# AmandineBtto/NeRAF

Measured on AMD Instinct MI355X. Metric: field-samples/sec (rays + RIR STFT bins), higher is better.
Workload: dtype f16; 1 GPU; RAF FurnishedRoom joint training step (BASELINE configs[2]): 4096 rays + 2048 RIR slices x 513 bins per GPU; radiance + grid refresh + ResNet3D + NAcF + STFT loss, backward, GradScaler + fused Adam...; rays_per_gpu=4096, slices_per_gpu=2048, global_rays=4096, global_slices=2048, parallelism=dp1, distinct_resident_batches=16, deterministic=True

## Files before the change

include/neraf_hip.h:

```cpp
#ifndef NERAF_HIP_H
#define NERAF_HIP_H

#include <stddef.h>
#include <stdint.h>

#ifdef __cplusplus
extern "C" {
#endif

typedef struct neraf_ctx neraf_ctx;
typedef void* neraf_stream_t;

enum {
  NERAF_OK = 0,
  NERAF_EINVAL = -1,
  NERAF_EHIP = -2,
  NERAF_ENOGPU = -3,
  NERAF_ESTATE = -4
};

#define NERAF_ABI_VERSION 1

int neraf_abi_version(void);
int neraf_ctx_create(neraf_ctx** out, int device);
// ... 238 lines not shown
                           const float* g_reg, float* d_pose, neraf_stream_t stream);

int neraf_loss_sum_scale(neraf_ctx* ctx, const float* const* terms, int n, const float* scale, float* out2, neraf_stream_t stream);
int neraf_vision_loss_finalize(neraf_ctx* ctx, const float* sums, const float* k3, float* out4, neraf_stream_t stream);
int neraf_vision_bwd_prologue(neraf_ctx* ctx, const float* u_rgb, const float* u_dens, const float* u_dist, const float* g_rgb,
                              const float* g_inter, const float* g_dist, size_t n_samples, float* d_rgb, float* d_dens, float* up3,
                              float* d_rays, size_t n_ray_floats, float* sums4, neraf_stream_t stream);

int neraf_cvt_f16_segments(neraf_ctx* ctx, const float* const* src, void* const* dst, const long long* len, int n,
                           neraf_stream_t stream);
int neraf_gather_f16(neraf_ctx* ctx, const float* const* src, const long long* src_len, int nsrc, const long long* index, void* dst,
                     long long n, neraf_stream_t stream);

int neraf_resnet3d_debug_locate(const neraf_resnet3d_desc* d, int kind, int index, size_t* offset, int* rows, int* cols);

uint32_t neraf_debug_fastdiv(uint32_t n, uint32_t d);

int neraf_fused_adam_chunk(void);
int neraf_grads_nonfinite(neraf_ctx* ctx, const void* table, const void* g_ptrs, const int* blk_tensor, const int* blk_chunk,
                          int n_blocks, float* found_inf, const void* const* g_ptrs_host, int n_ptrs, int found_is_zero,
                          neraf_stream_t stream);
int neraf_amp_update_scale(neraf_ctx* ctx, float* scale, int32_t* growth_tracker, const float* const* found_infs, int n,
                           double growth_factor, double backoff_factor, int growth_interval, int clear_flags, neraf_stream_t stream);
int neraf_fused_adam(neraf_ctx* ctx, const void* table, const void* g_ptrs, const int* blk_tensor, const int* blk_chunk,
                     int n_blocks, const float* group_lr, int n_groups, int n_tensors, double beta1, double beta2, double eps,
                     float* step, const float* grad_scale, const float* found_inf, neraf_stream_t stream);

int neraf_fused_adam_dual(neraf_ctx* ctx, const void* table, const void* g_ptrs, const int* blk_tensor, const int* blk_chunk,
                          int n_blocks, const float* group_lr, int n_groups, int n_tensors, double beta1, double beta2, double eps,
                          float* step, const float* grad_scale, const float* found_inf, const void* dual, const float* step0,
// ... 8 lines not shown
```

neraf_amd/_lib.py:

```python
from __future__ import annotations

import ctypes as C
import os
from typing import Dict, Optional

_HERE = os.path.dirname(os.path.abspath(__file__))
LIB_PATH = os.environ.get("NERAF_HIP_LIB") or os.path.join(_HERE, "libneraf_hip.so")

_lib: Optional[C.CDLL] = None
_ctxs: Dict[int, C.c_void_p] = {}

c_fpp = C.POINTER(C.c_void_p)


class GridDesc(C.Structure):
    _fields_ = [("n_levels", C.c_int), ("base_res", C.c_int), ("max_res", C.c_int), ("log2_hashmap_size", C.c_int),
                ("n_features", C.c_int)]


class ResnetDesc(C.Structure):
    _fields_ = [("grid_size", C.c_int), ("in_channels", C.c_int), ("n_features", C.c_int)]


class NacfDesc(C.Structure):
# ... 147 lines not shown
    "neraf_camera_apply": (C.c_int, [C.c_void_p, C.c_void_p, C.c_void_p, C.c_void_p, C.c_void_p, C.c_int, C.c_void_p, C.c_void_p, C.c_int,
                                     C.c_float, C.c_float, C.c_void_p, C.c_void_p]),
    "neraf_camera_apply_bwd": (C.c_int, [C.c_void_p, C.c_void_p, C.c_void_p, C.c_void_p, C.c_void_p, C.c_void_p, C.c_int, C.c_int, C.c_int,
                                         C.c_float, C.c_float, C.c_void_p, C.c_void_p, C.c_void_p]),
    "neraf_amp_update_scale": (C.c_int, [C.c_void_p, C.c_void_p, C.c_void_p, c_fpp, C.c_int, C.c_double, C.c_double, C.c_int, C.c_int,
                                         C.c_void_p]),
    "neraf_loss_sum_scale": (C.c_int, [C.c_void_p, c_fpp, C.c_int, C.c_void_p, C.c_void_p, C.c_void_p]),
    "neraf_vision_loss_finalize": (C.c_int, [C.c_void_p, C.c_void_p, C.c_void_p, C.c_void_p, C.c_void_p]),
    "neraf_vision_bwd_prologue": (C.c_int, [C.c_void_p] * 7 + [C.c_size_t, C.c_void_p, C.c_void_p, C.c_void_p, C.c_void_p, C.c_size_t,
                                            C.c_void_p, C.c_void_p]),
    "neraf_cvt_f16_segments": (C.c_int, [C.c_void_p, c_fpp, c_fpp, C.POINTER(C.c_longlong), C.c_int, C.c_void_p]),
    "neraf_gather_f16": (C.c_int, [C.c_void_p, c_fpp, C.POINTER(C.c_longlong), C.c_int, C.c_void_p, C.c_void_p, C.c_longlong, C.c_void_p]),
    "neraf_debug_fastdiv": (C.c_uint32, [C.c_uint32, C.c_uint32]),
    "neraf_resnet3d_debug_locate": (C.c_int, [C.POINTER(ResnetDesc), C.c_int, C.c_int, C.POINTER(C.c_size_t), C.POINTER(C.c_int),
                                              C.POINTER(C.c_int)]),
    "neraf_debug_conv_bn_relu_stage": (C.c_int, [C.c_void_p] + [C.c_int] * 7 + [C.c_void_p] * 11),
    "neraf_composite": (C.c_int, [C.c_void_p, C.c_void_p, C.c_void_p, C.c_void_p, C.c_int, C.c_int, C.c_int, C.c_void_p,
                                  C.c_void_p, C.c_void_p, C.c_void_p, C.c_void_p, C.c_void_p, C.c_size_t, C.c_void_p]),
}


def load() -> C.CDLL:
    global _lib
    if _lib is not None:
        return _lib
    if not os.path.exists(LIB_PATH):
        raise RuntimeError(
            f"{LIB_PATH} is missing: build it with `python -c 'import __graft_entry__ as g; g.build()'` "
            "(or `make -C neraf_amd/csrc`).  neraf_amd has no CPU / eager fallback by design.")
    lib = C.CDLL(LIB_PATH)
# ... 57 lines not shown
```

neraf_amd/csrc/gemm_f16.hip:

```cpp
#include "common.h"
#include <stdlib.h>
#include <type_traits>

namespace {

constexpr int BK = 64;

__device__ __forceinline__ float act_apply(float v, int act) {
  if (act == ACT_LEAKY) return v > 0.f ? v : 0.1f * v;
  if (act == ACT_TANH10) return 10.f * tanhf(v);
  if (act == ACT_RELU) return v > 0.f ? v : 0.f;
  return v;
}

template <bool BF> struct ET;
template <> struct ET<false> {
  typedef _Float16 s; typedef half8 v8; typedef half4 v4;
  static __device__ __forceinline__ f32x4 mfma(v8 a, v8 b, f32x4 c) { return __builtin_amdgcn_mfma_f32_16x16x32_f16(a, b, c, 0, 0, 0); }
};
template <> struct ET<true> {
  typedef __bf16 s; typedef bf16x8 v8; typedef bf16x4 v4;
  static __device__ __forceinline__ f32x4 mfma(v8 a, v8 b, f32x4 c) { return __builtin_amdgcn_mfma_f32_16x16x32_bf16(a, b, c, 0, 0, 0); }
};

// ... 818 lines not shown
  }
  return NERAF_OK;
}

constexpr int kStreamRows = 64;
constexpr int stream_slices(int n) { return n > 128 ? n / 128 : 1; }

__device__ __forceinline__ float row16_sum(float x) {
  x += __builtin_bit_cast(float, __builtin_amdgcn_mov_dpp(__builtin_bit_cast(int, x), 0xB1, 0xF, 0xF, true));
  x += __builtin_bit_cast(float, __builtin_amdgcn_mov_dpp(__builtin_bit_cast(int, x), 0x4E, 0xF, 0xF, true));
  x += __builtin_bit_cast(float, __builtin_amdgcn_mov_dpp(__builtin_bit_cast(int, x), 0x141, 0xF, 0xF, true));
  x += __builtin_bit_cast(float, __builtin_amdgcn_mov_dpp(__builtin_bit_cast(int, x), 0x140, 0xF, 0xF, true));
  return x;
}

template <int N, int K, bool STATS>
__global__ __launch_bounds__(512) void gemm_f16_nt_stream_kernel(GemmParams p, int nblocks, int nrg) {
  constexpr int R = kStreamRows, KB = K / 32;
  constexpr int CS = stream_slices(N), NW = N / CS, FNW = NW / 16;
  constexpr int CPRB = K / 8, SWZ = (CPRB - 1) & 15;
  constexpr int BCH = NW * CPRB / 512;
  constexpr int IC = 64, NPASS = NW / IC, FNP = IC / 16, IMG_LD = IC + 8, CPR = IC / 8, IMG_WAVE = 16 * IMG_LD * 2;
  static_assert(N * K <= 16384 && N % 64 == 0 && K % 64 == 0 && NW <= 128 && BCH >= 1, "B must fit 32 KiB of LDS");
  static_assert(8 * 2 * NW * 4 <= 8 * IMG_WAVE, "the statistics' reduction re-uses the result images");
  __shared__ __attribute__((aligned(16))) char bs[NW * K * 2];
  __shared__ __attribute__((aligned(16))) char img_all[8 * IMG_WAVE];

  const int tid = threadIdx.x;
  const int lane = tid & 63;
  const int wave = __builtin_amdgcn_readfirstlane(tid >> 6);
  const int g = wave >> 2, w4 = wave & 3;
  const int frow = lane & 15, fq = lane >> 4;
  int rg, cs;
  if (CS > 1 && (nrg & 7) == 0) { const int q = blockIdx.x >> 3; cs = q % CS; rg = (q / CS) * 8 + (blockIdx.x & 7); }
  else { rg = blockIdx.x / CS; cs = blockIdx.x - rg * CS; }
  const int n_w0 = cs * NW;
  const int nv = 2 * nrg;

// ... 105 lines not shown
    if (tid < 2 * NW) {
      const int which = tid / NW, col = tid - which * NW;
      float v = 0.f;
#pragma unroll
      for (int w = 0; w < 8; ++w) v += red[(w * 2 + which) * NW + col];
      float* dst = which ? p.colsumsq : p.colsum;
      if (dst) {
        if (p.stat_det) dst[(size_t)((2 * rg * R) >> 5) * p.stat_stride + n_w0 + col] = v;
        else atomicAdd(dst + (p.stat_rep > 1 ? (rg & (p.stat_rep - 1)) * p.stat_stride : 0) + n_w0 + col, v);
      }
    }
  }
}

static bool stream_qualifies(const GemmParams& p) {
  const bool nk = (p.N == 64 || p.N == 128 || p.N == 256) && (p.K == 64 || p.K == 128 || p.K == 256) && p.N * p.K <= 16384;
  return nk && p.Npad == p.N && p.conv.loader == 0 && p.ngroups <= 1 && !p.bf16 && (p.Mpad % kStreamRows) == 0 && p.C16 &&
         !p.bias && !p.act && !p.lmask && !p.C16T && !p.C32 && !p.alpha_dev && !p.bnb_x && !p.bnb_mask &&
         (!p.add16 || (p.ldadd % 4) == 0);
}

template <int N, int K>
int launch_stream_nk(neraf_ctx* ctx, const GemmParams& p, hipStream_t stream) {
  const int nblocks = p.Mpad / kStreamRows;
  constexpr int CS = stream_slices(N);
  int nrg = (ctx ? ctx->num_cus : 256) / CS;
  if (p.stream_max_wg > 0 && nrg > p.stream_max_wg / CS) nrg = p.stream_max_wg / CS;
  if (nrg > (nblocks + 1) / 2) nrg = (nblocks + 1) / 2;
  if (nrg < 1) nrg = 1;
  const int grid = nrg * CS;
  const double flops = p.alg_flops > 0.0 ? p.alg_flops : 2.0 * p.M * p.N * p.K;
  ProfScope prof(ctx, stream, N == 64 ? PROF_GEMM12864 : PROF_GEMM_WIDE, flops, 2.0 * p.M * p.N * p.K);
  if (p.colsum || p.colsumsq) hipLaunchKernelGGL((gemm_f16_nt_stream_kernel<N, K, true>), dim3(grid), dim3(512), 0, stream, p, nblocks, nrg);
  else hipLaunchKernelGGL((gemm_f16_nt_stream_kernel<N, K, false>), dim3(grid), dim3(512), 0, stream, p, nblocks, nrg);
  NERAF_HIP_CHECK(ctx, hipGetLastError());
  if (ctx && ctx->manifest) gemm_manifest(ctx, p, 0, 1, N, K, flops, false, true);
  return NERAF_OK;
}

int launch_stream(neraf_ctx* ctx, const GemmParams& p, hipStream_t stream) {
  switch (p.N * 1000 + p.K) {
    case 64064: return launch_stream_nk<64, 64>(ctx, p, stream);
    case 64128: return launch_stream_nk<64, 128>(ctx, p, stream);
    case 64256: return launch_stream_nk<64, 256>(ctx, p, stream);
    case 128064: return launch_stream_nk<128, 64>(ctx, p, stream);
    case 128128: return launch_stream_nk<128, 128>(ctx, p, stream);
    case 256064: return launch_stream_nk<256, 64>(ctx, p, stream);
  }
  return neraf_fail(ctx, NERAF_EINVAL, "gemm: shape outside the streaming body's");
}

struct WgDesc {
  const void* dy; const void* x; float* out;
  unsigned long long slab_off;
  int block_begin; int K;
  unsigned short cout, cin, cin_real, taps, din, tiles_n, splits;
  unsigned char dl, stride, ksize, loader; signed char pad; unsigned char mh, ai, r2, r3, r4;
};
static_assert(sizeof(WgDesc) == 64, "descriptor table must fit the 4 KiB kernel-argument segment");
constexpr int kMaxWg = 56;
struct WgTable { int n; int total_blocks; const half_t* zero_page; const float* alpha_dev; float* slab; int order; WgDesc d[kMaxWg]; };

// ... 744 lines not shown
```

neraf_amd/csrc/resnet3d.hip:

```cpp
#include "resnet3d_common.h"
#include <algorithm>

namespace {

__global__ __launch_bounds__(256) void grid_to_ndhwc8_kernel(const float* __restrict__ grid, size_t nvox, half_t* __restrict__ out) {
  const size_t v = (size_t)blockIdx.x * 256 + threadIdx.x;
  if (v >= nvox) return;
  half8 h;
#pragma unroll
  for (int c = 0; c < 7; ++c) h[c] = (half_t)grid[c * nvox + v];
  h[7] = (half_t)0.f;
  reinterpret_cast<half8*>(out)[v] = h;
}

__global__ __launch_bounds__(256) void grid_window_to_ndhwc8_kernel(const float* __restrict__ grid, size_t nvox, const unsigned long long* start,
                                                                   int n, half_t* __restrict__ out) {
  const int t = blockIdx.x * 256 + threadIdx.x;
  if (t >= n) return;
  const size_t v = (size_t)*start + t;
  if (v >= nvox) return;
  half8 h;
#pragma unroll
  for (int c = 0; c < 7; ++c) h[c] = (half_t)grid[c * nvox + v];
  h[7] = (half_t)0.f;
// ... 13 lines not shown
};

__global__ __launch_bounds__(256) void bn_update_running_all_kernel(RunTable t, const char* __restrict__ ws, float mom) {
  if (blockIdx.x == 0 && (int)threadIdx.x < t.n && t.nbt[threadIdx.x]) *t.nbt[threadIdx.x] += 1;
  const int idx = blockIdx.x * 256 + threadIdx.x;
  if (idx >= t.begin[t.n]) return;
  int lo = 0, hi = t.n - 1;
  while (lo < hi) { const int mid = (lo + hi + 1) >> 1; if (t.begin[mid] <= idx) lo = mid; else hi = mid - 1; }
  const int i = lo, c = idx - t.begin[i];
  const float* fin = reinterpret_cast<const float*>(ws + t.stat_off[i]);
  const float mean = fin[c], var = fin[t.cpad[i] + c];
  t.rmean[i][c] = (1.f - mom) * t.rmean[i][c] + mom * mean;
  t.rvar[i][c] = (1.f - mom) * t.rvar[i][c] + mom * var * t.unbias[i];
}

__global__ __launch_bounds__(256) void bn_relu_maxpool_kernel(BnSrc s, int din, int dout, size_t m_in, half_t* __restrict__ out,
                                                             unsigned char* __restrict__ arg) {
  __shared__ float sc[64], sh[64];
  if (threadIdx.x < 64) bn_scale_shift(s, threadIdx.x, 1.f / (float)m_in, sc[threadIdx.x], sh[threadIdx.x]);
  __syncthreads();
  const size_t total = cube(dout) * 8;
  const size_t idx = (size_t)blockIdx.x * 256 + threadIdx.x;
  if (idx >= total) return;
  const size_t vox = idx >> 3; const int c0 = (int)(idx & 7) * 8;
  const int x = (int)(vox % dout), y = (int)((vox / dout) % dout), z = (int)(vox / ((size_t)dout * dout));
  float best[8]; int at[8];
#pragma unroll
  for (int j = 0; j < 8; ++j) { best[j] = -3.0e38f; at[j] = 255; }
  for (int dz = -1; dz <= 1; ++dz) {
    const int iz = 2 * z + dz; if ((unsigned)iz >= (unsigned)din) continue;
    for (int dy = -1; dy <= 1; ++dy) {
      const int iy = 2 * y + dy; if ((unsigned)iy >= (unsigned)din) continue;
      for (int dx = -1; dx <= 1; ++dx) {
        const int ix = 2 * x + dx; if ((unsigned)ix >= (unsigned)din) continue;
        const half8 v = *reinterpret_cast<const half8*>(s.x + (((size_t)iz * din + iy) * din + ix) * 64 + c0);
        const int tap = (dz + 1) * 9 + (dy + 1) * 3 + (dx + 1);
#pragma unroll
        for (int j = 0; j < 8; ++j) {
          const float a = fmaxf(fmaf((float)v[j], sc[c0 + j], sh[c0 + j]), 0.f);
          if (a > best[j]) { best[j] = a; at[j] = tap; }
        }
      }
    }
  }
  if (arg) {
    unsigned long long packed = 0ull;
#pragma unroll
    for (int j = 0; j < 8; ++j) packed |= (unsigned long long)(best[j] > 0.f ? at[j] : 255) << (8 * j);
    *reinterpret_cast<unsigned long long*>(arg + vox * 64 + c0) = packed;
  }
  half8 o;
#pragma unroll
  for (int j = 0; j < 8; ++j) o[j] = (half_t)best[j];
  *reinterpret_cast<half8*>(out + vox * 64 + c0) = o;
}

__global__ __launch_bounds__(256) void avgpool_kernel(const half_t* __restrict__ x, int M, int C, float* __restrict__ feat) {
  __shared__ float part[32][65];
  const int chunk = threadIdx.x & 7, grp = threadIdx.x >> 3;
// ... 62 lines not shown
    *offset = kind == 0 ? L.a1[index] : kind == 1 ? L.a2[index] : L.out[index];
    *rows = (int)cube(c.dout); *cols = c.cout;
    return NERAF_OK;
  }
  if (kind == 7) { *offset = L.x0; *rows = (int)cube(A.S); *cols = 8; return NERAF_OK; }
  if (kind == 3) { *offset = L.act_pool; *rows = (int)cube(A.pooled); *cols = 64; return NERAF_OK; }
  if (kind == 4) { *offset = L.pool_arg; *rows = (int)cube(A.pooled); *cols = 64; return NERAF_OK; }
  if (kind == 5 || kind == 6) {
    if (index < 0 || index >= A.nconv) return NERAF_EINVAL;
    const ConvSpec& c = A.conv[index];
    if (kind == 5) { *offset = L.pre[index]; *rows = (int)cube(c.dout); *cols = c.cout; }
    else { *offset = L.fin[index]; *rows = 2; *cols = round_up(c.cout, 128); }
    return NERAF_OK;
  }
  return NERAF_EINVAL;
}

extern "C" int neraf_resnet3d_pack_weights(neraf_ctx* ctx, const neraf_resnet3d_desc* d, const float* const* conv_w, void* packed,
                                           neraf_stream_t stream) {
  Arch A; Layout L;
  if (make_arch(d, &A) || !conv_w || !packed) return neraf_fail(ctx, NERAF_EINVAL, "resnet3d_pack_weights: bad arguments");
  make_layout(A, &L);
  hipStream_t st = (hipStream_t)stream;
  PackTable t{};
  BrickTable bt{};
  unsigned long long acc = 0;
  int tiles = 0, max_run = 0;
  for (int i = 0; i < A.nconv; ++i) {
    const ConvSpec& c = A.conv[i];
    const int taps = c.k * c.k * c.k;
// ... 36 lines not shown
  neraf_node(ctx, "neraf_zero3_kernel | statistics accumulators", 0.0, 0.0, 256.0 + (double)L.stats_bytes + 4096.0);
  const size_t nvox = cube(A.S);
  const bool training = use_batch_stats != 0;
  if (win_cells > 0) {
    hipLaunchKernelGGL(grid_window_to_ndhwc8_kernel, dim3((unsigned)((win_cells + 255) / 256)), dim3(256), 0, st, grid, nvox,
                       reinterpret_cast<const unsigned long long*>(ws + L.win), win_cells, (half_t*)(ws + L.x0));
    neraf_node(ctx, "grid_window_to_ndhwc8_kernel | refresh window -> fp16 channels-last", 0.0, win_cells * 28.0, win_cells * 16.0);
  } else {
    hipLaunchKernelGGL(grid_to_ndhwc8_kernel, dim3((unsigned)((nvox + 255) / 256)), dim3(256), 0, st, grid, nvox, (half_t*)(ws + L.x0));
    neraf_node(ctx, "grid_to_ndhwc8_kernel | grid -> fp16 channels-last", 0.0, (double)nvox * 28.0, (double)nvox * 16.0);
  }
  if (int e = run_conv(ctx, st, A, L, 0, packed, ws, (const half_t*)(ws + L.x0))) return e;
  {
    const ConvSpec& c = A.conv[0];
    BnSrc s = bn_src_fwd(A, L, ws, bn, 0, use_batch_stats);
    const size_t total = cube(A.pooled) * 8;
    hipLaunchKernelGGL(bn_relu_maxpool_kernel, dim3((unsigned)((total + 255) / 256)), dim3(256), 0, st, s, c.dout, A.pooled,
                       cube(c.dout), (half_t*)(ws + L.act_pool), training ? (unsigned char*)(ws + L.pool_arg) : nullptr);
    NERAF_HIP_CHECK(ctx, hipGetLastError());
    neraf_node(ctx, "bn_relu_maxpool_kernel | stem BatchNorm + ReLU + 3x3x3/2 max-pool", 0.0, (double)cube(c.dout) * 64 * 2.0,
               (double)cube(A.pooled) * 64 * (training ? 3.0 : 2.0));
  }
  const half_t* x = (const half_t*)(ws + L.act_pool);
  for (int b = 0; b < A.nblock; ++b) {
    const BlockSpec& B = A.block[b];
    const int i0 = B.conv[0], i1 = B.conv[1], i2 = B.conv[2];
    const ConvSpec &c0 = A.conv[i0], &c1 = A.conv[i1], &c2 = A.conv[i2];
    if (int e = run_conv(ctx, st, A, L, i0, packed, ws, x)) return e;
    BnApplyArgs a{};
    a.a = bn_src_fwd(A, L, ws, bn, i0, use_batch_stats);
    a.M = (int)cube(c0.dout); a.Mpad = (int)rows_pad(c0.dout); a.C = c0.cout; a.relu = 1; a.out = (half_t*)(ws + L.a1[b]);
    if (int e = run_bn_apply(ctx, st, a)) return e;
// ... 73 lines not shown
```

neraf_amd/csrc/resnet3d_bwd.hip:

```cpp
#include "resnet3d_common.h"
#include <algorithm>
#include <mutex>
#include <stddef.h>
#include <stdlib.h>
#include <string.h>
#include <unordered_map>

namespace {

struct PackTTable {
  int n;
  const float* src[kMaxConv];
  int tile_begin[kMaxConv + 1];
  unsigned long long dst_off[kMaxConv];
  int cout[kMaxConv], cin[kMaxConv], taps[kMaxConv], kcols[kMaxConv], nrows[kMaxConv];
};

__global__ __launch_bounds__(256) void pack_dgrad_weights_kernel(PackTTable t, char* __restrict__ packed) {
  extern __shared__ half_t brick[];
  int lo = 0, hi = t.n - 1;
  const int bid = blockIdx.x;
  while (lo < hi) { const int mid = (lo + hi + 1) >> 1; if (t.tile_begin[mid] <= bid) lo = mid; else hi = mid - 1; }
  const int i = lo;
  const int tile = bid - t.tile_begin[i];
// ... 296 lines not shown
        else if (recorded) cs->unsettled = (unsigned)__popcll(bad);
        cs->passes = valid ? passes_in + 1u : 1u;
        cs->dfeat_bad = dfeat_bad ? 1u : 0u;
        cs->magic = kChainMagic;
      }
    }
  }
  const float k = S / (float)M;
  const size_t total = (size_t)Mpad * C;
  for (size_t idx = (size_t)blockIdx.x * 256 + threadIdx.x; idx < total; idx += (size_t)gridDim.x * 256) {
    const int row = (int)(idx / C), c = (int)(idx % C);
    g[idx] = (half_t)(row < M ? dfeat[c] * k : 0.f);
  }
}

__global__ __launch_bounds__(256) void maxpool_bwd_gather_kernel(const unsigned char* __restrict__ arg, int din, int dout,
                                                                const half_t* __restrict__ g, half_t* __restrict__ dpost, size_t rows_pad_in) {
  const size_t idx = (size_t)blockIdx.x * 256 + threadIdx.x;
  if (idx >= rows_pad_in * 8) return;
  const size_t vox = idx >> 3; const int c0 = (int)(idx & 7) * 8;
  float acc[8];
#pragma unroll
  for (int j = 0; j < 8; ++j) acc[j] = 0.f;
  if (vox < cube(din)) {
    const int ix = (int)(vox % din), iy = (int)((vox / din) % din), iz = (int)(vox / ((size_t)din * din));
    int oz[2], tz[2], oy[2], ty[2], ox[2], tx[2];
    auto wins = [&](int i, int (&o)[2], int (&tp)[2]) {
      if ((i & 1) == 0) { o[0] = i >> 1; tp[0] = 1; return 1; }
      o[0] = (i - 1) >> 1; tp[0] = 2;
      if (((i + 1) >> 1) < dout) { o[1] = (i + 1) >> 1; tp[1] = 0; return 2; }
      return 1;
    };
    const int nz = wins(iz, oz, tz), ny = wins(iy, oy, ty), nx = wins(ix, ox, tx);
    for (int a = 0; a < nz; ++a)
      for (int b = 0; b < ny; ++b)
        for (int c = 0; c < nx; ++c) {
          const size_t ov = ((size_t)oz[a] * dout + oy[b]) * dout + ox[c];
          const unsigned tap = (unsigned)(tz[a] * 9 + ty[b] * 3 + tx[c]);
          const unsigned long long am = *reinterpret_cast<const unsigned long long*>(arg + ov * 64 + c0);
          const half8 gv = *reinterpret_cast<const half8*>(g + ov * 64 + c0);
#pragma unroll
          for (int j = 0; j < 8; ++j)
            if (((am >> (8 * j)) & 0xffu) == tap) acc[j] += (float)gv[j];
        }
  }
  half8 o;
#pragma unroll
  for (int j = 0; j < 8; ++j) o[j] = (half_t)acc[j];
  *reinterpret_cast<half8*>(dpost + vox * 64 + c0) = o;
}

__global__ void set_f32x2_kernel(float* p, float a, float b) { if (threadIdx.x == 0 && blockIdx.x == 0) { p[0] = a; p[1] = b; } }
__global__ void set_u64_kernel(unsigned long long* p, unsigned long long v) { if (threadIdx.x == 0 && blockIdx.x == 0) p[0] = v; }

__global__ __launch_bounds__(256) void stem_w_relayout_kernel(const float* __restrict__ W, float* __restrict__ Wt) {
  const int idx = blockIdx.x * 256 + threadIdx.x;
  if (idx >= 125 * 8 * 64) return;
  const int co = idx & 63, c = (idx >> 6) & 7, tap = idx >> 9;
  Wt[idx] = c < 7 ? W[((size_t)co * 7 + c) * 125 + tap] : 0.f;
}

__global__ __launch_bounds__(256) void stem_dgrid_kernel(const half_t* __restrict__ dy, const float* __restrict__ Wt, int S, int dout,
                                                        const unsigned long long* __restrict__ start_dev, int n, int nch,
                                                        const float* __restrict__ inv_scale, float* __restrict__ dgrid) {
// ... 328 lines not shown
      items[n_items++] = wgrad_item(c, Bk.ds, dyds, x_in, k0);
      if (int e = conv_dgrad(c, i0, dy0, nullptr, g_next)) return e;
      if (int e = conv_dgrad(c, Bk.ds, dyds, g_next, g_next)) return e;
    } else {
      const bool fg = b > 0 && A.block[b - 1].ds < 0 && fuse_bn_sums(A.conv[A.block[b - 1].conv[2]]);
      if (int e = conv_dgrad(c, i0, dy0, gm, g_next, fg ? A.block[b - 1].conv[2] : -1, fg ? (const half_t*)(ws + L.out[b - 1]) : nullptr)) return e;
      g_sums_done = fg;
    }
    half_t* t = g; g = g_next; g_next = t;
    k_g = k0;
  }
  {
    const ConvSpec& c0 = A.conv[0];
    half_t* dpost = (half_t*)(bws + B.dpost);
    const size_t rp = rows_pad(c0.dout);
    hipLaunchKernelGGL(maxpool_bwd_gather_kernel, dim3((unsigned)((rp * 8 + 255) / 256)), dim3(256), 0, st,
                       (const unsigned char*)(ws + L.pool_arg), c0.dout, A.pooled, g, dpost, rp);
    NERAF_HIP_CHECK(ctx, hipGetLastError());
    neraf_node(ctx, "maxpool_bwd_gather_kernel | max-pool routing", 0.0, (double)cube(A.pooled) * 64 * 3.0, (double)rp * 64 * 2.0);
    half_t* dy0 = (half_t*)(bws + B.dy[0]);
    const int k_s = new_k(k_g);
    if (int e = bn_backward(c, 0, dpost, nullptr, nullptr, dy0, nullptr, k_g, k_s, -1)) return e;
    items[n_items++] = wgrad_item(c, 0, dy0, (const half_t*)(ws + L.x0), k_s);
    if (n_cells > 0) {
      float* Wt = (float*)(bws + B.wtmp);
      hipLaunchKernelGGL(stem_w_relayout_kernel, dim3((125 * 8 * 64 + 255) / 256), dim3(256), 0, st, conv_w[0], Wt);
      hipLaunchKernelGGL(stem_dgrid_kernel, dim3((n_cells + 3) / 4), dim3(256), 0, st, dy0, Wt, A.S, c0.dout,
                         reinterpret_cast<const unsigned long long*>(bws + B.scale + 64), n_cells, n_ch, c.inv(k_s), dgrid_cells);
      NERAF_HIP_CHECK(ctx, hipGetLastError());
      neraf_node(ctx, "stem_w_relayout_kernel | W[co][c][tap] -> Wt[tap][c][co]", 0.0, 125.0 * 7 * 64 * 4, 125.0 * 8 * 64 * 4);
      neraf_node(ctx, "stem_dgrid_kernel | grid gradient of the refresh window", 2.0 * n_cells * (125.0 / 8.0) * 64 * n_ch, (double)n_cells * (125.0 / 8.0) * 128.0,
// ... 98 lines not shown
  make_bwd_layout(A, &B);
  const char* bws = (const char*)bwd_workspace;
  NERAF_HIP_CHECK(ctx, hipStreamSynchronize((hipStream_t)stream));
  ChainState cs;
  NERAF_HIP_CHECK(ctx, hipMemcpy(&cs, bws + B.chain, sizeof(cs), hipMemcpyDeviceToHost));
  std::vector<unsigned> am((size_t)n * kAmaxRep * kAmaxStride);
  NERAF_HIP_CHECK(ctx, hipMemcpy(am.data(), bws + B.amax, am.size() * 4, hipMemcpyDeviceToHost));
  for (int t = 0; t < n; ++t) {
    unsigned mx = 0;
    for (int r = 0; r < kAmaxRep; ++r) mx = std::max(mx, am[((size_t)t * kAmaxRep + r) * kAmaxStride]);
    float f; memcpy(&f, &mx, 4);
    e_out[t] = cs.magic == kChainMagic ? cs.e[t] : 0;
    amax_out[t] = f;
  }
  if (info2) { info2[0] = (int32_t)cs.unsettled; info2[1] = (int32_t)cs.passes; }
  return NERAF_OK;
}

extern "C" int neraf_debug_conv_bn_relu_stage(neraf_ctx* ctx, int cin, int cin_real, int cout, int k, int stride, int pad, int din,
                                              const void* x_f16, const float* w, const float* gamma, const float* beta, const float* g,
                                              void* y_f16, float* dx, float* dw, float* dgamma, float* dbeta, neraf_stream_t stream) {
  hipStream_t st = (hipStream_t)stream;
  Arch A{};
  A.S = din; A.nconv = 1; A.nblock = 0; A.pooled = din; A.final_edge = din; A.n_features = 1024;
  const int dout = (din + 2 * pad - k) / stride + 1;
  A.conv[0] = ConvSpec{cin, cout, k, stride, pad, din, dout, cin_real};
  Layout L{}; BwdLayout B{};
  make_layout(A, &L);
  make_bwd_layout(A, &B);
  const size_t act = std::max(rows_pad(dout) * (size_t)cout, rows_pad(din) * (size_t)cin) * 2 + 256;
// ... 55 lines not shown
```

neraf_amd/csrc/resnet3d_common.h:

```cpp
#pragma once
#include "common.h"

namespace {

constexpr int kMaxConv = 56;
struct ConvSpec { int cin, cout, k, stride, pad, din, dout; int cin_real; };
struct BlockSpec { int conv[3]; int ds; int planes; };

struct Arch {
  int S;
  int nconv;
  ConvSpec conv[64];
  int nblock;
  BlockSpec block[16];
  int pooled;
  int final_edge;
  int n_features;
};

int make_arch(const neraf_resnet3d_desc* d, Arch* A) {
  if (!d || d->in_channels != 7 || (d->n_features != 1024 && d->n_features != 2048) ||
      (d->grid_size != 128 && d->grid_size != 64 && d->grid_size != 256)) return NERAF_EINVAL;
  A->S = d->grid_size;
  A->n_features = d->n_features;
// ... 400 lines not shown
  if (c.k == 1 && c.stride == 1) {
    g.conv.loader = 0;
  } else {
    g.conv.loader = c.cin == 8 ? 2 : 1;
    g.conv.din = c.din; g.conv.dout = c.dout; g.conv.stride = c.stride; g.conv.pad = c.pad; g.conv.ksize = c.k; g.conv.cin = c.cin;
    g.conv.zero_page = (const half_t*)(ws + L.zero_page);
  }
  if (int e = launch_gemm_f16(ctx, g, st)) return e;
  if (det) {
    run_slot_sum(st, stats, det_slots(c), cpad, 1.f / (float)M, 1, (float*)(ws + L.fin[ci]));
    NERAF_HIP_CHECK(ctx, hipGetLastError());
  }
  return NERAF_OK;
}

inline int run_bn_apply(neraf_ctx* ctx, hipStream_t st, const BnApplyArgs& a) {
  const size_t total = (size_t)a.Mpad * (a.C >> 3);
  long blocks = (long)((total + 255) / 256);
  if (blocks > 2048) blocks = 2048;
  hipLaunchKernelGGL(bn_apply_kernel, dim3((unsigned)blocks), dim3(256), (size_t)4 * a.C * sizeof(float), st, a);
  if (ctx && ctx->manifest) {
    char nm[96];
    snprintf(nm, sizeof(nm), "bn_apply_kernel | M=%d C=%d%s", a.M, a.C, a.r.x ? " + bn(downsample)" : (a.res ? " + residual" : ""));
    neraf_node(ctx, nm, 0.0, (double)a.M * a.C * 2.0 * ((a.r.x || a.res) ? 2 : 1), (double)a.Mpad * a.C * 2.0);
  }
  NERAF_HIP_CHECK(ctx, hipGetLastError());
  return NERAF_OK;
}


}
```

Before: 267.5 million field-samples/s.

## Retile ResNet3D BN-apply, maxpool fwd/bwd, and widen streaming GEMM shapes

```diff
diff --git a/include/neraf_hip.h b/include/neraf_hip.h
--- a/include/neraf_hip.h
+++ b/include/neraf_hip.h
@@ -276,6 +276,13 @@
 
 int neraf_resnet3d_debug_locate(const neraf_resnet3d_desc* d, int kind, int index, size_t* offset, int* rows, int* cols);
 
+int neraf_debug_bn_apply(neraf_ctx* ctx, const void* x, const float* const* bn5, int rep, const void* xr, const float* const* bn5_r,
+                         int rep_r, const void* res, int M, int Mpad, int C, int relu, float* fin_w, float* fin_w_r, void* out,
+                         int form, neraf_stream_t stream);
+int neraf_debug_maxpool_fwd(neraf_ctx* ctx, const void* x, const float* const* bn5, int rep, int din, void* out, void* arg,
+                            neraf_stream_t stream);
+int neraf_debug_maxpool_bwd(neraf_ctx* ctx, const void* arg, const void* g, int din, void* dpost, neraf_stream_t stream);
+
 uint32_t neraf_debug_fastdiv(uint32_t n, uint32_t d);
 
 int neraf_fused_adam_chunk(void);
diff --git a/neraf_amd/_lib.py b/neraf_amd/_lib.py
--- a/neraf_amd/_lib.py
+++ b/neraf_amd/_lib.py
@@ -185,6 +185,10 @@
     "neraf_debug_fastdiv": (C.c_uint32, [C.c_uint32, C.c_uint32]),
     "neraf_resnet3d_debug_locate": (C.c_int, [C.POINTER(ResnetDesc), C.c_int, C.c_int, C.POINTER(C.c_size_t), C.POINTER(C.c_int),
                                               C.POINTER(C.c_int)]),
+    "neraf_debug_bn_apply": (C.c_int, [C.c_void_p, C.c_void_p, c_fpp, C.c_int, C.c_void_p, c_fpp, C.c_int, C.c_void_p, C.c_int, C.c_int, C.c_int,
+                                       C.c_int, C.c_void_p, C.c_void_p, C.c_void_p, C.c_int, C.c_void_p]),
+    "neraf_debug_maxpool_fwd": (C.c_int, [C.c_void_p, C.c_void_p, c_fpp, C.c_int, C.c_int, C.c_void_p, C.c_void_p, C.c_void_p]),
+    "neraf_debug_maxpool_bwd": (C.c_int, [C.c_void_p, C.c_void_p, C.c_void_p, C.c_int, C.c_void_p, C.c_void_p]),
     "neraf_debug_conv_bn_relu_stage": (C.c_int, [C.c_void_p] + [C.c_int] * 7 + [C.c_void_p] * 11),
     "neraf_composite": (C.c_int, [C.c_void_p, C.c_void_p, C.c_void_p, C.c_void_p, C.c_int, C.c_int, C.c_int, C.c_void_p,
                                   C.c_void_p, C.c_void_p, C.c_void_p, C.c_void_p, C.c_void_p, C.c_size_t, C.c_void_p]),
diff --git a/neraf_amd/csrc/gemm_f16.hip b/neraf_amd/csrc/gemm_f16.hip
--- a/neraf_amd/csrc/gemm_f16.hip
+++ b/neraf_amd/csrc/gemm_f16.hip
@@ -856,14 +856,14 @@
   return x;
 }
 
-template <int N, int K, bool STATS>
+template <int N, int K, int CS, bool STATS>
 __global__ __launch_bounds__(512) void gemm_f16_nt_stream_kernel(GemmParams p, int nblocks, int nrg) {
   constexpr int R = kStreamRows, KB = K / 32;
-  constexpr int CS = stream_slices(N), NW = N / CS, FNW = NW / 16;
+  constexpr int NW = N / CS, FNW = NW / 16;
   constexpr int CPRB = K / 8, SWZ = (CPRB - 1) & 15;
   constexpr int BCH = NW * CPRB / 512;
   constexpr int IC = 64, NPASS = NW / IC, FNP = IC / 16, IMG_LD = IC + 8, CPR = IC / 8, IMG_WAVE = 16 * IMG_LD * 2;
-  static_assert(N * K <= 16384 && N % 64 == 0 && K % 64 == 0 && NW <= 128 && BCH >= 1, "B must fit 32 KiB of LDS");
+  static_assert(NW * K <= 16384 && NW % 64 == 0 && K % 64 == 0 && NW <= 128 && BCH >= 1, "a workgroup's slice of B must fit 32 KiB of LDS");
   static_assert(8 * 2 * NW * 4 <= 8 * IMG_WAVE, "the statistics' reduction re-uses the result images");
   __shared__ __attribute__((aligned(16))) char bs[NW * K * 2];
   __shared__ __attribute__((aligned(16))) char img_all[8 * IMG_WAVE];
@@ -999,16 +999,15 @@
 }
 
 static bool stream_qualifies(const GemmParams& p) {
-  const bool nk = (p.N == 64 || p.N == 128 || p.N == 256) && (p.K == 64 || p.K == 128 || p.K == 256) && p.N * p.K <= 16384;
+  const bool nk = (p.N == 64 || p.N == 128 || p.N == 256) && (p.K == 64 || p.K == 128 || p.K == 256) && p.N * p.K <= 32768;
   return nk && p.Npad == p.N && p.conv.loader == 0 && p.ngroups <= 1 && !p.bf16 && (p.Mpad % kStreamRows) == 0 && p.C16 &&
          !p.bias && !p.act && !p.lmask && !p.C16T && !p.C32 && !p.alpha_dev && !p.bnb_x && !p.bnb_mask &&
          (!p.add16 || (p.ldadd % 4) == 0);
 }
 
-template <int N, int K>
+template <int N, int K, int CS = stream_slices(N)>
 int launch_stream_nk(neraf_ctx* ctx, const GemmParams& p, hipStream_t stream) {
   const int nblocks = p.Mpad / kStreamRows;
-  constexpr int CS = stream_slices(N);
   int nrg = (ctx ? ctx->num_cus : 256) / CS;
   if (p.stream_max_wg > 0 && nrg > p.stream_max_wg / CS) nrg = p.stream_max_wg / CS;
   if (nrg > (nblocks + 1) / 2) nrg = (nblocks + 1) / 2;
@@ -1016,8 +1015,8 @@
   const int grid = nrg * CS;
   const double flops = p.alg_flops > 0.0 ? p.alg_flops : 2.0 * p.M * p.N * p.K;
   ProfScope prof(ctx, stream, N == 64 ? PROF_GEMM12864 : PROF_GEMM_WIDE, flops, 2.0 * p.M * p.N * p.K);
-  if (p.colsum || p.colsumsq) hipLaunchKernelGGL((gemm_f16_nt_stream_kernel<N, K, true>), dim3(grid), dim3(512), 0, stream, p, nblocks, nrg);
-  else hipLaunchKernelGGL((gemm_f16_nt_stream_kernel<N, K, false>), dim3(grid), dim3(512), 0, stream, p, nblocks, nrg);
+  if (p.colsum || p.colsumsq) hipLaunchKernelGGL((gemm_f16_nt_stream_kernel<N, K, CS, true>), dim3(grid), dim3(512), 0, stream, p, nblocks, nrg);
+  else hipLaunchKernelGGL((gemm_f16_nt_stream_kernel<N, K, CS, false>), dim3(grid), dim3(512), 0, stream, p, nblocks, nrg);
   NERAF_HIP_CHECK(ctx, hipGetLastError());
   if (ctx && ctx->manifest) gemm_manifest(ctx, p, 0, 1, N, K, flops, false, true);
   return NERAF_OK;
@@ -1031,6 +1030,8 @@
     case 128064: return launch_stream_nk<128, 64>(ctx, p, stream);
     case 128128: return launch_stream_nk<128, 128>(ctx, p, stream);
     case 256064: return launch_stream_nk<256, 64>(ctx, p, stream);
+    case 128256: return launch_stream_nk<128, 256, 2>(ctx, p, stream);
+    case 256128: return launch_stream_nk<256, 128, 2>(ctx, p, stream);
   }
   return neraf_fail(ctx, NERAF_EINVAL, "gemm: shape outside the streaming body's");
 }
diff --git a/neraf_amd/csrc/resnet3d.hip b/neraf_amd/csrc/resnet3d.hip
--- a/neraf_amd/csrc/resnet3d.hip
+++ b/neraf_amd/csrc/resnet3d.hip
@@ -51,35 +51,58 @@
   t.rvar[i][c] = (1.f - mom) * t.rvar[i][c] + mom * var * t.unbias[i];
 }
 
+inline unsigned pool_blocks(int dout) { return (unsigned)((cube(dout) * 8 + 255) / 256); }
+
 __global__ __launch_bounds__(256) void bn_relu_maxpool_kernel(BnSrc s, int din, int dout, size_t m_in, half_t* __restrict__ out,
                                                              unsigned char* __restrict__ arg) {
-  __shared__ float sc[64], sh[64];
+  __shared__ __attribute__((aligned(16))) float sc[64], sh[64];
+  const size_t total = cube(dout) * 8;
+  const size_t idx = (size_t)blockIdx.x * 256 + threadIdx.x;
+  const bool active = idx < total;
+  const size_t vox = active ? idx >> 3 : 0; const int c0 = (int)(idx & 7) * 8;
+  const int x = (int)(vox % dout), y = (int)((vox / dout) % dout), z = (int)(vox / ((size_t)dout * dout));
+  bool okz[3], oky[3], okx[3];
+  size_t offy[3], offx[3];
+#pragma unroll
+  for (int d = 0; d < 3; ++d) {
+    okz[d] = (unsigned)(2 * z + d - 1) < (unsigned)din; oky[d] = (unsigned)(2 * y + d - 1) < (unsigned)din; okx[d] = (unsigned)(2 * x + d - 1) < (unsigned)din;
+    offy[d] = (size_t)min(max(2 * y + d - 1, 0), din - 1) * din * 64;
+    offx[d] = (size_t)min(max(2 * x + d - 1, 0), din - 1) * 64 + c0;
+  }
+  auto load_plane = [&](int d, uint4 (&pl)[9]) {
+    const half_t* base = s.x + (size_t)min(max(2 * z + d - 1, 0), din - 1) * din * din * 64;
+#pragma unroll
+    for (int t = 0; t < 9; ++t) pl[t] = *reinterpret_cast<const uint4*>(base + offy[t / 3] + offx[t % 3]);
+  };
+  uint4 pa[9], pb[9];
+  load_plane(0, pa);
+  load_plane(1, pb);
   if (threadIdx.x < 64) bn_scale_shift(s, threadIdx.x, 1.f / (float)m_in, sc[threadIdx.x], sh[threadIdx.x]);
   __syncthreads();
-  const size_t total = cube(dout) * 8;
-  const size_t idx = (size_t)blockIdx.x * 256 + threadIdx.x;
-  if (idx >= total) return;
-  const size_t vox = idx >> 3; const int c0 = (int)(idx & 7) * 8;
-  const int x = (int)(vox % dout), y = (int)((vox / dout) % dout), z = (int)(vox / ((size_t)dout * dout));
+  if (!active) return;
+  float scv[8], shv[8];
+  *reinterpret_cast<f32x4*>(scv) = *reinterpret_cast<const f32x4*>(sc + c0); *reinterpret_cast<f32x4*>(scv + 4) = *reinterpret_cast<const f32x4*>(sc + c0 + 4);
+  *reinterpret_cast<f32x4*>(shv) = *reinterpret_cast<const f32x4*>(sh + c0); *reinterpret_cast<f32x4*>(shv + 4) = *reinterpret_cast<const f32x4*>(sh + c0 + 4);
   float best[8]; int at[8];
 #pragma unroll
   for (int j = 0; j < 8; ++j) { best[j] = -3.0e38f; at[j] = 255; }
-  for (int dz = -1; dz <= 1; ++dz) {
-    const int iz = 2 * z + dz; if ((unsigned)iz >= (unsigned)din) continue;
-    for (int dy = -1; dy <= 1; ++dy) {
-      const int iy = 2 * y + dy; if ((unsigned)iy >= (unsigned)din) continue;
-      for (int dx = -1; dx <= 1; ++dx) {
-        const int ix = 2 * x + dx; if ((unsigned)ix >= (unsigned)din) continue;
-        const half8 v = *reinterpret_cast<const half8*>(s.x + (((size_t)iz * din + iy) * din + ix) * 64 + c0);
-        const int tap = (dz + 1) * 9 + (dy + 1) * 3 + (dx + 1);
-#pragma unroll
-        for (int j = 0; j < 8; ++j) {
-          const float a = fmaxf(fmaf((float)v[j], sc[c0 + j], sh[c0 + j]), 0.f);
-          if (a > best[j]) { best[j] = a; at[j] = tap; }
-        }
+  auto reduce_plane = [&](int d, const uint4 (&pl)[9]) {
+#pragma unroll
+    for (int t = 0; t < 9; ++t) {
+      if (!(okz[d] && oky[t / 3] && okx[t % 3])) continue;
+      const half8 v = *reinterpret_cast<const half8*>(&pl[t]);
+      const int tap = d * 9 + t;
+#pragma unroll
+      for (int j = 0; j < 8; ++j) {
+        const float a = fmaxf(fmaf((float)v[j], scv[j], shv[j]), 0.f);
+        if (a > best[j]) { best[j] = a; at[j] = tap; }
       }
     }
-  }
+  };
+  reduce_plane(0, pa);
+  load_plane(2, pa);
+  reduce_plane(1, pb);
+  reduce_plane(2, pa);
   if (arg) {
     unsigned long long packed = 0ull;
 #pragma unroll
@@ -172,6 +195,41 @@
     return NERAF_OK;
   }
   return NERAF_EINVAL;
+}
+
+static BnSrc debug_bn_src(const void* x, const float* const* bn5, int rep, int C, float* fin_w) {
+  BnSrc s{};
+  s.read_mode = bn_stat_read_mode();
+  s.x = (const half_t*)x;
+  s.stats = bn5[0]; s.fin_w = bn5[0] ? fin_w : nullptr;
+  s.gamma = bn5[1]; s.beta = bn5[2]; s.rmean = bn5[3]; s.rvar = bn5[4];
+  s.cpad = round_up(C, 128); s.rep = rep;
+  return s;
+}
+
+extern "C" int neraf_debug_bn_apply(neraf_ctx* ctx, const void* x, const float* const* bn5, int rep, const void* xr,
+                                    const float* const* bn5_r, int rep_r, const void* res, int M, int Mpad, int C, int relu,
+                                    float* fin_w, float* fin_w_r, void* out, int form, neraf_stream_t stream) {
+  if (!x || !bn5 || !out || (xr && (!bn5_r || res)) || M < 1 || Mpad < M || Mpad % 128 || C < 8 || C % 8 || form < 0 || form > 1 ||
+      rep < 1 || rep > 16 || (xr && (rep_r < 1 || rep_r > 16)) || ((rep > 1 || (xr && rep_r > 1)) && 2 * round_up(C, 128) > kStatStride))
+    return neraf_fail(ctx, NERAF_EINVAL, "debug_bn_apply: bad arguments");
+  BnApplyArgs a{};
+  a.a = debug_bn_src(x, bn5, rep, C, fin_w);
+  if (xr) a.r = debug_bn_src(xr, bn5_r, rep_r, C, fin_w_r);
+  a.res = (const half_t*)res;
+  a.M = M; a.Mpad = Mpad; a.C = C; a.relu = relu; a.out = (half_t*)out;
+  return run_bn_apply(ctx, (hipStream_t)stream, a, form);
+}
+
+extern "C" int neraf_debug_maxpool_fwd(neraf_ctx* ctx, const void* x, const float* const* bn5, int rep, int din, void* out, void* arg,
+                                       neraf_stream_t stream) {
+  if (!x || !bn5 || !out || din < 2 || din > 256 || rep < 1 || rep > 16) return neraf_fail(ctx, NERAF_EINVAL, "debug_maxpool_fwd: bad arguments");
+  const int dout = (din - 1) / 2 + 1;
+  BnSrc s = debug_bn_src(x, bn5, rep, 64, nullptr);
+  hipLaunchKernelGGL(bn_relu_maxpool_kernel, dim3(pool_blocks(dout)), dim3(256), 0, (hipStream_t)stream, s, din, dout, cube(din),
+                     (half_t*)out, (unsigned char*)arg);
+  NERAF_HIP_CHECK(ctx, hipGetLastError());
+  return NERAF_OK;
 }
 
 extern "C" int neraf_resnet3d_pack_weights(neraf_ctx* ctx, const neraf_resnet3d_desc* d, const float* const* conv_w, void* packed,
@@ -238,8 +296,7 @@
   {
     const ConvSpec& c = A.conv[0];
     BnSrc s = bn_src_fwd(A, L, ws, bn, 0, use_batch_stats);
-    const size_t total = cube(A.pooled) * 8;
-    hipLaunchKernelGGL(bn_relu_maxpool_kernel, dim3((unsigned)((total + 255) / 256)), dim3(256), 0, st, s, c.dout, A.pooled,
+    hipLaunchKernelGGL(bn_relu_maxpool_kernel, dim3(pool_blocks(A.pooled)), dim3(256), 0, st, s, c.dout, A.pooled,
                        cube(c.dout), (half_t*)(ws + L.act_pool), training ? (unsigned char*)(ws + L.pool_arg) : nullptr);
     NERAF_HIP_CHECK(ctx, hipGetLastError());
     neraf_node(ctx, "bn_relu_maxpool_kernel | stem BatchNorm + ReLU + 3x3x3/2 max-pool", 0.0, (double)cube(c.dout) * 64 * 2.0,
diff --git a/neraf_amd/csrc/resnet3d_bwd.hip b/neraf_amd/csrc/resnet3d_bwd.hip
--- a/neraf_amd/csrc/resnet3d_bwd.hip
+++ b/neraf_amd/csrc/resnet3d_bwd.hip
@@ -334,40 +334,87 @@
   }
 }
 
+constexpr int kGatherCz = 2, kGatherCy = 4, kGatherCx = 4;
+constexpr int kGatherWin = (kGatherCz + 1) * (kGatherCy + 1) * (kGatherCx + 1);
+static_assert(kGatherCz * kGatherCy * kGatherCx * 8 == 256, "one cell-chunk per thread");
+
+inline unsigned gather_blocks(int din) {
+  const int nc = (din + 1) / 2;
+  return (unsigned)(((nc + kGatherCz - 1) / kGatherCz) * ((nc + kGatherCy - 1) / kGatherCy) * ((nc + kGatherCx - 1) / kGatherCx));
+}
+
 __global__ __launch_bounds__(256) void maxpool_bwd_gather_kernel(const unsigned char* __restrict__ arg, int din, int dout,
                                                                 const half_t* __restrict__ g, half_t* __restrict__ dpost, size_t rows_pad_in) {
-  const size_t idx = (size_t)blockIdx.x * 256 + threadIdx.x;
-  if (idx >= rows_pad_in * 8) return;
-  const size_t vox = idx >> 3; const int c0 = (int)(idx & 7) * 8;
-  float acc[8];
-#pragma unroll
-  for (int j = 0; j < 8; ++j) acc[j] = 0.f;
-  if (vox < cube(din)) {
-    const int ix = (int)(vox % din), iy = (int)((vox / din) % din), iz = (int)(vox / ((size_t)din * din));
-    int oz[2], tz[2], oy[2], ty[2], ox[2], tx[2];
-    auto wins = [&](int i, int (&o)[2], int (&tp)[2]) {
-      if ((i & 1) == 0) { o[0] = i >> 1; tp[0] = 1; return 1; }
-      o[0] = (i - 1) >> 1; tp[0] = 2;
-      if (((i + 1) >> 1) < dout) { o[1] = (i + 1) >> 1; tp[1] = 0; return 2; }
-      return 1;
-    };
-    const int nz = wins(iz, oz, tz), ny = wins(iy, oy, ty), nx = wins(ix, ox, tx);
-    for (int a = 0; a < nz; ++a)
-      for (int b = 0; b < ny; ++b)
-        for (int c = 0; c < nx; ++c) {
-          const size_t ov = ((size_t)oz[a] * dout + oy[b]) * dout + ox[c];
-          const unsigned tap = (unsigned)(tz[a] * 9 + ty[b] * 3 + tx[c]);
-          const unsigned long long am = *reinterpret_cast<const unsigned long long*>(arg + ov * 64 + c0);
-          const half8 gv = *reinterpret_cast<const half8*>(g + ov * 64 + c0);
-#pragma unroll
-          for (int j = 0; j < 8; ++j)
-            if (((am >> (8 * j)) & 0xffu) == tap) acc[j] += (float)gv[j];
-        }
-  }
-  half8 o;
-#pragma unroll
-  for (int j = 0; j < 8; ++j) o[j] = (half_t)acc[j];
-  *reinterpret_cast<half8*>(dpost + vox * 64 + c0) = o;
+  __shared__ unsigned long long s_arg[kGatherWin * 8];
+  __shared__ uint4 s_g[kGatherWin * 8];
+  const int tid = threadIdx.x;
+  const int nc = (din + 1) / 2;
+  const int nbx = (nc + kGatherCx - 1) / kGatherCx, nby = (nc + kGatherCy - 1) / kGatherCy;
+  const int bx = blockIdx.x % nbx, by = (blockIdx.x / nbx) % nby, bz = blockIdx.x / (nbx * nby);
+  const int oz0 = bz * kGatherCz, oy0 = by * kGatherCy, ox0 = bx * kGatherCx;
+  {
+    constexpr int kSt = (kGatherWin * 8 + 255) / 256;
+    unsigned long long am_s[kSt]; uint4 g_s[kSt]; bool inside[kSt];
+#pragma unroll
+    for (int k = 0; k < kSt; ++k) {
+      const int e = min(k * 256 + tid, kGatherWin * 8 - 1);
+      const int w = e >> 3;
+      const int oz = oz0 + w / ((kGatherCx + 1) * (kGatherCy + 1)), oy = oy0 + (w / (kGatherCx + 1)) % (kGatherCy + 1), ox = ox0 + w % (kGatherCx + 1);
+      inside[k] = oz < dout && oy < dout && ox < dout;
+      const size_t ov = ((size_t)min(oz, dout - 1) * dout + min(oy, dout - 1)) * dout + min(ox, dout - 1);
+      am_s[k] = *reinterpret_cast<const unsigned long long*>(arg + ov * 64 + (e & 7) * 8);
+      g_s[k] = *reinterpret_cast<const uint4*>(g + ov * 64 + (e & 7) * 8);
+    }
+#pragma unroll
+    for (int k = 0; k < kSt; ++k) {
+      const int e = k * 256 + tid;
+      if (e < kGatherWin * 8) { s_arg[e] = inside[k] ? am_s[k] : ~0ull; s_g[e] = inside[k] ? g_s[k] : make_uint4(0u, 0u, 0u, 0u); }
+    }
+  }
+  if (blockIdx.x == 0) {
+    const size_t first = cube(din) * 8, total = rows_pad_in * 8;
+    for (size_t e = first + tid; e < total; e += 256) reinterpret_cast<uint4*>(dpost)[e] = make_uint4(0u, 0u, 0u, 0u);
+  }
+  __syncthreads();
+  const int ch = tid & 7, lc = tid >> 3;
+  const int lx = lc % kGatherCx, ly = (lc / kGatherCx) % kGatherCy, lz = lc / (kGatherCx * kGatherCy);
+  unsigned long long am[8];
+  half8 gv[8];
+#pragma unroll
+  for (int k = 0; k < 8; ++k) {
+    const int w = ((lz + (k >> 2)) * (kGatherCy + 1) + ly + ((k >> 1) & 1)) * (kGatherCx + 1) + lx + (k & 1);
+    am[k] = s_arg[w * 8 + ch];
+    const uint4 raw = s_g[w * 8 + ch];
+    gv[k] = *reinterpret_cast<const half8*>(&raw);
+  }
+#pragma unroll
+  for (int pz = 0; pz < 2; ++pz)
+#pragma unroll
+    for (int py = 0; py < 2; ++py)
+#pragma unroll
+      for (int px = 0; px < 2; ++px) {
+        const int iz = 2 * (oz0 + lz) + pz, iy = 2 * (oy0 + ly) + py, ix = 2 * (ox0 + lx) + px;
+        if (iz >= din || iy >= din || ix >= din) continue;
+        float acc[8];
+#pragma unroll
+        for (int j = 0; j < 8; ++j) acc[j] = 0.f;
+#pragma unroll
+        for (int a = 0; a <= pz; ++a)
+#pragma unroll
+          for (int b = 0; b <= py; ++b)
+#pragma unroll
+            for (int c = 0; c <= px; ++c) {
+              const unsigned tap = (unsigned)((pz ? 2 - 2 * a : 1) * 9 + (py ? 2 - 2 * b : 1) * 3 + (px ? 2 - 2 * c : 1));
+              const int k = a * 4 + b * 2 + c;
+#pragma unroll
+              for (int j = 0; j < 8; ++j)
+                if (((am[k] >> (8 * j)) & 0xffu) == tap) acc[j] += (float)gv[k][j];
+            }
+        half8 o;
+#pragma unroll
+        for (int j = 0; j < 8; ++j) o[j] = (half_t)acc[j];
+        *reinterpret_cast<half8*>(dpost + (((size_t)iz * din + iy) * din + ix) * 64 + ch * 8) = o;
+      }
 }
 
 __global__ void set_f32x2_kernel(float* p, float a, float b) { if (threadIdx.x == 0 && blockIdx.x == 0) { p[0] = a; p[1] = b; } }
@@ -726,7 +773,7 @@
     const ConvSpec& c0 = A.conv[0];
     half_t* dpost = (half_t*)(bws + B.dpost);
     const size_t rp = rows_pad(c0.dout);
-    hipLaunchKernelGGL(maxpool_bwd_gather_kernel, dim3((unsigned)((rp * 8 + 255) / 256)), dim3(256), 0, st,
+    hipLaunchKernelGGL(maxpool_bwd_gather_kernel, dim3(gather_blocks(c0.dout)), dim3(256), 0, st,
                        (const unsigned char*)(ws + L.pool_arg), c0.dout, A.pooled, g, dpost, rp);
     NERAF_HIP_CHECK(ctx, hipGetLastError());
     neraf_node(ctx, "maxpool_bwd_gather_kernel | max-pool routing", 0.0, (double)cube(A.pooled) * 64 * 3.0, (double)rp * 64 * 2.0);
@@ -855,6 +902,14 @@
     amax_out[t] = f;
   }
   if (info2) { info2[0] = (int32_t)cs.unsettled; info2[1] = (int32_t)cs.passes; }
+  return NERAF_OK;
+}
+
+extern "C" int neraf_debug_maxpool_bwd(neraf_ctx* ctx, const void* arg, const void* g, int din, void* dpost, neraf_stream_t stream) {
+  if (!arg || !g || !dpost || din < 2 || din > 256) return neraf_fail(ctx, NERAF_EINVAL, "debug_maxpool_bwd: bad arguments");
+  hipLaunchKernelGGL(maxpool_bwd_gather_kernel, dim3(gather_blocks(din)), dim3(256), 0, (hipStream_t)stream, (const unsigned char*)arg,
+                     din, (din - 1) / 2 + 1, (const half_t*)g, (half_t*)dpost, rows_pad(din));
+  NERAF_HIP_CHECK(ctx, hipGetLastError());
   return NERAF_OK;
 }
 
diff --git a/neraf_amd/csrc/resnet3d_common.h b/neraf_amd/csrc/resnet3d_common.h
--- a/neraf_amd/csrc/resnet3d_common.h
+++ b/neraf_amd/csrc/resnet3d_common.h
@@ -438,14 +438,74 @@
   return NERAF_OK;
 }
 
-inline int run_bn_apply(neraf_ctx* ctx, hipStream_t st, const BnApplyArgs& a) {
+template <int U>
+__global__ __launch_bounds__(256) void bn_apply_tile_kernel(BnApplyArgs p) {
+  __shared__ __attribute__((aligned(16))) float sc[64], sh[64], scr[64], shr[64];
+  const int tid = threadIdx.x;
+  const int c_base = blockIdx.y * 64, c0 = (tid & 7) * 8;
+  const int m0 = blockIdx.x * (32 * U) + (tid >> 3);
+  const float inv_m = 1.f / (float)p.M;
+  const half_t* second = p.r.x ? p.r.x : p.res;
+  half8 x[U], rr[U];
+#pragma unroll
+  for (int it = 0; it < U; ++it) {
+    const int row = m0 + it * 32;
+    if (row < p.M) {
+      const size_t off = (size_t)row * p.C + c_base + c0;
+      x[it] = *reinterpret_cast<const half8*>(p.a.x + off);
+      if (second) rr[it] = *reinterpret_cast<const half8*>(second + off);
+    }
+  }
+  if (tid < 64) bn_scale_shift(p.a, c_base + tid, inv_m, sc[tid], sh[tid]);
+  else if (tid < 128 && p.r.x) bn_scale_shift(p.r, c_base + tid - 64, inv_m, scr[tid - 64], shr[tid - 64]);
+  __syncthreads();
+  float scv[8], shv[8], scrv[8], shrv[8];
+  *reinterpret_cast<f32x4*>(scv) = *reinterpret_cast<const f32x4*>(sc + c0); *reinterpret_cast<f32x4*>(scv + 4) = *reinterpret_cast<const f32x4*>(sc + c0 + 4);
+  *reinterpret_cast<f32x4*>(shv) = *reinterpret_cast<const f32x4*>(sh + c0); *reinterpret_cast<f32x4*>(shv + 4) = *reinterpret_cast<const f32x4*>(sh + c0 + 4);
+  if (p.r.x) {
+    *reinterpret_cast<f32x4*>(scrv) = *reinterpret_cast<const f32x4*>(scr + c0); *reinterpret_cast<f32x4*>(scrv + 4) = *reinterpret_cast<const f32x4*>(scr + c0 + 4);
+    *reinterpret_cast<f32x4*>(shrv) = *reinterpret_cast<const f32x4*>(shr + c0); *reinterpret_cast<f32x4*>(shrv + 4) = *reinterpret_cast<const f32x4*>(shr + c0 + 4);
+  }
+#pragma unroll
+  for (int it = 0; it < U; ++it) {
+    const int row = m0 + it * 32;
+    half8 o;
+    if (row < p.M) {
+#pragma unroll
+      for (int j = 0; j < 8; ++j) {
+        float v = fmaf((float)x[it][j], scv[j], shv[j]);
+        if (p.r.x) v += fmaf((float)rr[it][j], scrv[j], shrv[j]);
+        else if (p.res) v += (float)rr[it][j];
+        if (p.relu) v = fmaxf(v, 0.f);
+        o[j] = (half_t)v;
+      }
+    } else {
+#pragma unroll
+      for (int j = 0; j < 8; ++j) o[j] = (half_t)0.f;
+    }
+    *reinterpret_cast<half8*>(p.out + (size_t)row * p.C + c_base + c0) = o;
+  }
+}
+
+constexpr size_t kBnTileMinChunks = (size_t)1 << 16;
+constexpr int kBnTileU = 2;
+inline bool bn_tile_fits(const BnApplyArgs& a) { return a.C % 64 == 0 && a.Mpad % (32 * kBnTileU) == 0; }
+
+inline int run_bn_apply(neraf_ctx* ctx, hipStream_t st, const BnApplyArgs& a, int form = -1) {
   const size_t total = (size_t)a.Mpad * (a.C >> 3);
-  long blocks = (long)((total + 255) / 256);
-  if (blocks > 2048) blocks = 2048;
-  hipLaunchKernelGGL(bn_apply_kernel, dim3((unsigned)blocks), dim3(256), (size_t)4 * a.C * sizeof(float), st, a);
+  if (form == 1 && !bn_tile_fits(a)) return neraf_fail(ctx, NERAF_EINVAL, "bn_apply: the tile form needs C % 64 == 0 and Mpad % 64 == 0");
+  const bool tile = form < 0 ? (total >= kBnTileMinChunks && bn_tile_fits(a)) : form == 1;
+  if (tile) {
+    hipLaunchKernelGGL(bn_apply_tile_kernel<kBnTileU>,dim3((unsigned)(a.Mpad / (32 * kBnTileU)), (unsigned)(a.C / 64)), dim3(256), 0, st, a);
+  } else {
+    long blocks = (long)((total + 255) / 256);
+    if (blocks > 2048) blocks = 2048;
+    hipLaunchKernelGGL(bn_apply_kernel, dim3((unsigned)blocks), dim3(256), (size_t)4 * a.C * sizeof(float), st, a);
+  }
   if (ctx && ctx->manifest) {
     char nm[96];
-    snprintf(nm, sizeof(nm), "bn_apply_kernel | M=%d C=%d%s", a.M, a.C, a.r.x ? " + bn(downsample)" : (a.res ? " + residual" : ""));
+    snprintf(nm, sizeof(nm), "%s | M=%d C=%d%s", tile ? "bn_apply_tile_kernel" : "bn_apply_kernel", a.M, a.C,
+             a.r.x ? " + bn(downsample)" : (a.res ? " + residual" : ""));
     neraf_node(ctx, nm, 0.0, (double)a.M * a.C * 2.0 * ((a.r.x || a.res) ? 2 : 1), (double)a.Mpad * a.C * 2.0);
   }
   NERAF_HIP_CHECK(ctx, hipGetLastError());
```

After: 274.3 million field-samples/s (median of 6 runs). 1.03x the previous value.
